# ivanalberico/End-To-End-Self-Supervised-SLAM

Hardware: AMD Instinct MI355X
Metric: online refinement steps/sec @640x480, seq_len=60 (higher is better)
Workload: dtype f32

## Files before the change

### end-to-end-self-supervised-slam_amd/csrc/conv.hip

```cpp
#include <type_traits>

#include "e2e_common.h"

typedef float f4v __attribute__((ext_vector_type(4)));
typedef float f16v __attribute__((ext_vector_type(16)));

#define CBK 16

enum { ACT_NONE = 0, ACT_RELU = 1, ACT_ELU = 2, ACT_DISP = 3 };

struct ConvArgs {
    const float* src0;
    const float* src1;
    const float* w;
    const float* scale;
    const float* shift;
    const float* res;
    float* out;
    int B, Hs, Ws;
    int Cin, C1, up;
    int Hd, Wd;
    int Ncols, ldw;
    int KH, KW, stride, pad, pad_mode;
    int off;
// ... 1733 lines not shown
        __syncthreads();
        store_chunk();
        __syncthreads();
        if (c + 1 < c_end) load_chunk(c + 1);
        constexpr int QB = 4, NQ = 32 / QB;
        float av[2][QB], bv[2][QB][3];
        auto read_q = [&](int set, int qt) {
#pragma unroll
            for (int j = 0; j < QB; ++j) {
                const int ks = QB * qt + j, q0 = (ks >> 2) * 10 + 2 * (ks & 3);
                av[set][j] = ap[2 * ks * 32];
#pragma unroll
                for (int t = 0; t < 3; ++t) bv[set][j][t] = bp[(q0 + t) * 32];
            }
        };
        auto pin_q = [&](int set) {
#pragma unroll
            for (int j = 0; j < QB; ++j) {
                asm volatile("" : "+v"(av[set][j]));
#pragma unroll
                for (int t = 0; t < 3; ++t) asm volatile("" : "+v"(bv[set][j][t]));
            }
        };
        read_q(0, 0);
#pragma unroll
        for (int qt = 0; qt < NQ; ++qt) {
            if (qt + 1 < NQ) read_q((qt + 1) & 1, qt + 1);
            __builtin_amdgcn_sched_barrier(0);
            pin_q(qt & 1);
            __builtin_amdgcn_sched_barrier(0);
#pragma unroll
            for (int j = 0; j < QB; ++j) {
#pragma unroll
                for (int t = 0; t < 3; ++t) acc[t] = __builtin_amdgcn_mfma_f32_32x32x2f32(av[qt & 1][j], bv[qt & 1][j][t], acc[t], 0, 0, 0);
                if (BIAS && want_bias) accb = __builtin_amdgcn_mfma_f32_32x32x2f32(av[qt & 1][j], one, accb, 0, 0, 0);
            }
            __builtin_amdgcn_sched_barrier(0);
        }
    }
    float* slab = a.slabs + (int64_t)blockIdx.z * a.Mpad * a.Npad;
#pragma unroll
    for (int t = 0; t < 3; ++t)
#pragma unroll
        for (int r = 0; r < 16; ++r) {
            const int m = co0 + (r & 3) + 8 * (r >> 2) + 4 * kh_;
            slab[(int64_t)m * a.Npad + (wave * 3 + t) * a.Cin + ci0 + l32] = acc[t][r];
        }
    if (BIAS && want_bias && l32 == 0) {
#pragma unroll
        for (int r = 0; r < 16; ++r) slab[(int64_t)(co0 + (r & 3) + 8 * (r >> 2) + 4 * kh_) * a.Npad + 9 * a.Cin] = accb[r];
    }
}

template <int ZL>
__device__ __forceinline__ void wgrad_reduce_group(const float* __restrict__ slabs, int S, int Mpad, int Npad, int Cout, int Cin, int KH, int KW, int has_bias,
                                                   float* __restrict__ dw, float* __restrict__ dbias, int accumulate, const float* __restrict__ scale,
                                                   int64_t base, int e, int w, f4v (*part)[64]) {
    const int Kconv = KH * KW * Cin, Ng = Kconv + (has_bias ? 1 : 0);
    const int nq = (Ng + 3) / 4;
    const int64_t totalq = (int64_t)Cout * nq;
    const int64_t slab_q = (int64_t)Mpad * Npad / 4;
    const f4v zero = {0.f, 0.f, 0.f, 0.f};
    const int64_t q = base + e;
    const bool on = q < totalq;
    const int m = on ? (int)(q / nq) : 0, n = on ? (int)(q - (int64_t)m * nq) * 4 : 0;
    const f4v* src = (const f4v*)(slabs + (int64_t)m * Npad + n);
    f4v sacc = zero;
    int z = w;
    for (; z + 3 * ZL < S; z += 4 * ZL) {
        f4v v[4];
#pragma unroll
        for (int j = 0; j < 4; ++j) v[j] = on ? src[(int64_t)(z + ZL * j) * slab_q] : zero;
#pragma unroll
        for (int j = 0; j < 4; ++j) sacc += v[j];
    }
    for (; z < S; z += ZL) sacc += on ? src[(int64_t)z * slab_q] : zero;
    part[w][e] = sacc;
    __syncthreads();
    if (w == 0 && on) {
        f4v t = part[0][e];
#pragma unroll
        for (int j = 1; j < ZL; ++j) t += part[j][e];
        if (scale) t *= scale[m];
#pragma unroll
        for (int k = 0; k < 4; ++k) {
            const int nn = n + k;
            if (nn < Kconv) {
                const int tap = nn / Cin, ci = nn - tap * Cin, kh = tap / KW, kw = tap - kh * KW;
                float* d = dw + (((int64_t)m * Cin + ci) * KH + kh) * KW + kw;
                *d = accumulate ? *d + t[k] : t[k];
            } else if (nn == Kconv && dbias) {
                dbias[m] = accumulate ? dbias[m] + t[k] : t[k];
            }
        }
    }
    __syncthreads();
}

template <int ZL>
__global__ __launch_bounds__(64 * ZL) void k_wgrad_reduce(const float* __restrict__ slabs, int S, int Mpad, int Npad, int Cout, int Cin,
                                                         int KH, int KW, int has_bias, float* __restrict__ dw, float* __restrict__ dbias,
                                                         int accumulate, const float* __restrict__ scale) {
    __shared__ f4v part[ZL][64];
    const int64_t totalq = (int64_t)Cout * ((KH * KW * Cin + (has_bias ? 1 : 0) + 3) / 4);
    for (int64_t base = (int64_t)blockIdx.x * 64; base < totalq; base += (int64_t)gridDim.x * 64)
        wgrad_reduce_group<ZL>(slabs, S, Mpad, Npad, Cout, Cin, KH, KW, has_bias, dw, dbias, accumulate, scale, base, threadIdx.x & 63, threadIdx.x >> 6, part);
}

__global__ __launch_bounds__(512) void k_wgrad_reduce_batched(const e2e_wgrad_reduce_desc* __restrict__ d, int n, long long total_items) {
    __shared__ f4v part[8][64];
    const int e = threadIdx.x & 63, w = threadIdx.x >> 6;
    for (long long item = blockIdx.x; item < total_items; item += gridDim.x) {
        int lo = 0, hi = n - 1;
        while (lo < hi) {
            const int mid = (lo + hi + 1) >> 1;
            if (d[mid].first_item <= item) lo = mid; else hi = mid - 1;
        }
        const e2e_wgrad_reduce_desc D = d[lo];
        const long long local = item - D.first_item;
        if (D.zl == 8)
            wgrad_reduce_group<8>(D.slabs, D.S, D.Mpad, D.Npad, D.Cout, D.Cin, D.KH, D.KW, D.has_bias, D.dw, D.dbias, D.accumulate, D.scale, local * 64, e, w, part);
        else
            wgrad_reduce_group<2>(D.slabs, D.S, D.Mpad, D.Npad, D.Cout, D.Cin, D.KH, D.KW, D.has_bias, D.dw, D.dbias, D.accumulate, D.scale,
                                  (local * 4 + (w >> 1)) * 64, e, w & 1, part + 2 * (w >> 1));
    }
}

__global__ __launch_bounds__(256) void k_weight_layouts(const float* __restrict__ w, int Cout, int Cin, int KH, int KW,
                                                        float* __restrict__ wf, int ldf, float* __restrict__ wb, int ldb) {
    const int64_t total = (int64_t)Cout * Cin * KH * KW;
    for (int64_t i = (int64_t)blockIdx.x * 256 + threadIdx.x; i < total; i += (int64_t)gridDim.x * 256) {
        int64_t t = i;
        const int kw = (int)(t % KW); t /= KW;
        const int kh = (int)(t % KH); t /= KH;
        const int ci = (int)(t % Cin); t /= Cin;
        const int co = (int)t;
        const float v = w[i];
        if (wf) wf[((int64_t)(kh * KW + kw) * Cin + ci) * ldf + co] = v;
        if (wb) wb[((int64_t)(kh * KW + kw) * Cout + co) * ldb + ci] = v;
    }
}

__global__ __launch_bounds__(256) void k_weight_layouts_batched(const long long* __restrict__ desc) {
    const long long* d = desc + (int64_t)blockIdx.y * 10;
    const float* __restrict__ w = (const float*)d[0];
    float* __restrict__ wf = (float*)d[1];
    float* __restrict__ wb = (float*)d[2];
    const int Cout = (int)d[3], Cin = (int)d[4], KH = (int)d[5], KW = (int)d[6], ldf = (int)d[7], ldb = (int)d[8];
    const float* __restrict__ bsc = (const float*)d[9];
    const int T = KH * KW;
    constexpr int TMAX = 9, TS = 32;
    __shared__ float tile[TMAX][TS + 1][TS + 1];
    if (T > TMAX) {
        const int64_t total = (int64_t)Cout * Cin * T;
        for (int64_t i = (int64_t)blockIdx.x * 256 + threadIdx.x; i < total; i += (int64_t)gridDim.x * 256) {
            const int tap = (int)(i % T);
            const int64_t r = i / T;
            const int ci = (int)(r % Cin), co = (int)(r / Cin);
            const float v = w[i];
            if (wf) wf[((int64_t)tap * Cin + ci) * ldf + co] = v;
            if (wb) wb[((int64_t)tap * Cout + co) * ldb + ci] = bsc ? v * bsc[co] : v;
        }
        return;
    }
    const int nct = (Cout + TS - 1) / TS, nit = (Cin + TS - 1) / TS;
    for (int t = blockIdx.x; t < nct * nit; t += gridDim.x) {
        const int co0 = (t / nit) * TS, ci0 = (t % nit) * TS;
        const int nci = min(TS, Cin - ci0), nco = min(TS, Cout - co0);
        const int row = nci * T;
        for (int e = threadIdx.x; e < nco * row; e += 256) {
            const int co_l = e / row, rem = e - co_l * row;
            const int ci_l = rem / T, tap = rem - ci_l * T;
            tile[tap][co_l][ci_l] = w[((int64_t)(co0 + co_l) * Cin + ci0) * T + rem];
        }
        __syncthreads();
        if (wf)
            for (int e = threadIdx.x; e < T * nci * nco; e += 256) {
                const int co_l = e % nco, r = e / nco;
                const int ci_l = r % nci, tap = r / nci;
                wf[((int64_t)tap * Cin + ci0 + ci_l) * ldf + co0 + co_l] = tile[tap][co_l][ci_l];
            }
        if (wb)
            for (int e = threadIdx.x; e < T * nco * nci; e += 256) {
                const int ci_l = e % nci, r = e / nci;
                const int co_l = r % nco, tap = r / nco;
                wb[((int64_t)tap * Cout + co0 + co_l) * ldb + ci0 + ci_l] = bsc ? tile[tap][co_l][ci_l] * bsc[co0 + co_l] : tile[tap][co_l][ci_l];
            }
        __syncthreads();
    }
}

__global__ __launch_bounds__(256) void k_act_bwd(const float* __restrict__ dy, const float* __restrict__ y, const float* __restrict__ scale,
                                                 float* __restrict__ dz, int64_t n, int C, int act, int accumulate) {
    for (int64_t i = (int64_t)blockIdx.x * 256 + threadIdx.x; i < n; i += (int64_t)gridDim.x * 256) {
        float g = dy[i];
        const float v = y[i];
        if (act == ACT_RELU) g = v > 0.f ? g : 0.f;
        else if (act == ACT_ELU) g = v > 0.f ? g : g * (v + 1.f);
        else if (act == ACT_DISP) { const float s = (v - 0.01f) * 0.1f; g = g * 10.f * s * (1.f - s); }
        if (scale) g *= scale[i % C];
        dz[i] = accumulate ? dz[i] + g : g;
    }
}

__global__ __launch_bounds__(256) void k_gather_adjoint(const float* __restrict__ dxp, int B, int Hs, int Ws, int Cin, int C1, int up,
                                                        int pp, float* __restrict__ d0, float* __restrict__ d1, int acc0, int acc1,
                                                        const float* __restrict__ x0, int act0, const float* __restrict__ x1, int act1) {
    const int Hp = Hs + 2 * pp, Wp = Ws + 2 * pp, C2 = Cin - C1, Hl = Hs / up, Wl = Ws / up;
    const int64_t n0 = (int64_t)B * Hl * Wl * C1, n1 = (int64_t)B * Hs * Ws * C2;
    for (int64_t i = (int64_t)blockIdx.x * 256 + threadIdx.x; i < n0 + n1; i += (int64_t)gridDim.x * 256) {
        const bool first = i < n0;
        int64_t t = first ? i : i - n0;
        const int Cx = first ? C1 : C2, Hx = first ? Hl : Hs, Wx = first ? Wl : Ws, u = first ? up : 1;
        const int c = (int)(t % Cx); t /= Cx;
        const int x = (int)(t % Wx); t /= Wx;
        const int y = (int)(t % Hx); t /= Hx;
        const int b = (int)t;
        const int cc = first ? c : C1 + c;
        float s = 0.f;
        for (int dy = 0; dy < u; ++dy)
            for (int dx = 0; dx < u; ++dx) {
                const int fy = y * u + dy, fx = x * u + dx;
                int ys[3] = {fy + pp, -1, -1}, xs[3] = {fx + pp, -1, -1};
                if (pp) {
                    if (fy == 1) ys[1] = 0;
                    if (fy == Hs - 2) ys[2] = Hp - 1;
                    if (fx == 1) xs[1] = 0;
                    if (fx == Ws - 2) xs[2] = Wp - 1;
                }
                for (int iy = 0; iy < 3; ++iy)
                    for (int ix = 0; ix < 3; ++ix)
                        if (ys[iy] >= 0 && xs[ix] >= 0) s += dxp[(((int64_t)b * Hp + ys[iy]) * Wp + xs[ix]) * Cin + cc];
            }
        float* d = first ? d0 + i : d1 + (i - n0);
        const int acc = first ? acc0 : acc1;
        if (first ? act0 : act1) s *= act_deriv(first ? x0[i] : x1[i - n0], first ? act0 : act1);
        *d = acc ? *d + s : s;
    }
}

__global__ __launch_bounds__(256) void k_gather_adjoint4(const float* __restrict__ dxp, int B, int Hs, int Ws, int Cin, int C1, int up,
// ... 281 lines not shown
            a.act == ACT_NONE) {
            a.ksplit = 4; a.cps = a.Cin / cb; a.cls_rows = Nc;
            dim3 g((unsigned)(4 * ((Nc + c.bm - 1) / c.bm)), (unsigned)((a.Ncols + c.bn - 1) / c.bn), 4u);
            launch_tile<TR>(a, cb, c, g, st);
            hipLaunchKernelGGL(k_conv_splitk_epilogue_cls, dim3(egrid(total / 4)), dim3(256), 0, st, workspace, Nc, a.B, a.Hd, a.Wd, a.Ncols, a.KH, a.KW, a.off,
                               a.res, a.out, a.xin, a.dact, a.pre);
            return;
        }
        dim3 g((unsigned)(4 * ((Nc + c.bm - 1) / c.bm)), (unsigned)((a.Ncols + c.bn - 1) / c.bn));
        launch_tile<TR>(a, cb, c, g, st);
        return;
    }
    const GemmCfg c = choose_cfg(Ntot, a.Ncols, K, cb, workspace != nullptr, force);
    if (c.S < 0 && workspace && vec == 4 && K % cb == 0 && a.Cin % cb == 0) {
        launch_streamk<TR>(a, cb, -c.S, workspace_all, st);
        return;
    }
    if (c.S > 1) {
        const int nchunks = (K + cb - 1) / cb;
        a.cps = (nchunks + c.S - 1) / c.S;
        const int Sz = (nchunks + a.cps - 1) / a.cps;
        a.ksplit = Sz;
        if (Sz > 1) {
            dim3 g((unsigned)((Ntot + c.bm - 1) / c.bm), (unsigned)((a.Ncols + c.bn - 1) / c.bn), (unsigned)Sz);
            launch_tile<TR>(a, cb, c, g, st);
            const int64_t total = Ntot * a.Ncols;
            if (a.Ncols % 4 == 0 && total < (1ll << 31))
                hipLaunchKernelGGL(k_conv_splitk_epilogue4, dim3(egrid(total / 4)), dim3(256), 0, st, workspace, Sz, (unsigned)(total / 4), a.Ncols, a.scale, a.shift,
                                   a.res, a.out, a.act, a.xin, a.dact, a.pre);
            else
                hipLaunchKernelGGL(k_conv_splitk_epilogue, dim3(egrid(total)), dim3(256), 0, st, workspace, Sz, total, a.Ncols, a.scale, a.shift, a.res, a.out, a.act, a.xin, a.dact, a.pre);
            return;
        }
        a.ksplit = 1; a.cps = 0;
    }
    dim3 g((unsigned)((Ntot + c.bm - 1) / c.bm), (unsigned)((a.Ncols + c.bn - 1) / c.bn));
    launch_tile<TR>(a, cb, c, g, st);
}

extern "C" {

int e2e_conv_weight_layouts(const float* w, int Cout, int Cin, int KH, int KW, float* w_fwd, int ld_fwd, float* w_bwd,
                            int ld_bwd, void* stream) {
    E2E_REQUIRE(w && Cout > 0 && Cin > 0 && KH > 0 && KW > 0 && (w_fwd || w_bwd), E2E_ERR_ARG, "e2e_conv_weight_layouts: bad argument");
    E2E_REQUIRE((!w_fwd || (ld_fwd >= Cout && ld_fwd % 4 == 0)) && (!w_bwd || (ld_bwd >= Cin && ld_bwd % 4 == 0)), E2E_ERR_ARG,
                "e2e_conv_weight_layouts: leading dimensions must cover the columns and be multiples of 4");
    hipLaunchKernelGGL(k_weight_layouts, dim3(egrid((int64_t)Cout * Cin * KH * KW)), dim3(256), 0, (hipStream_t)stream, w, Cout, Cin, KH,
                       KW, w_fwd, ld_fwd, w_bwd, ld_bwd);
    E2E_LAUNCH_CHECK("e2e_conv_weight_layouts");
    return E2E_OK;
}

int e2e_conv_weight_layouts_batched(const long long* desc, int nlayers, void* stream) {
    E2E_REQUIRE(desc && nlayers > 0 && nlayers <= 65535, E2E_ERR_ARG, "e2e_conv_weight_layouts_batched: bad argument");
    hipLaunchKernelGGL(k_weight_layouts_batched, dim3(256, nlayers), dim3(256), 0, (hipStream_t)stream, desc);
    E2E_LAUNCH_CHECK("e2e_conv_weight_layouts_batched");
    return E2E_OK;
}

int64_t e2e_conv2d_splitk_workspace_floats(int64_t rows, int cols, int K);
int64_t e2e_conv2d_bwd_data_workspace_floats(int B, int Hd, int Wd, int cols, int K, int stride) {
    const int64_t plain = e2e_conv2d_splitk_workspace_floats((int64_t)B * Hd * Wd, cols, K);
    if (stride != 2) return plain;
    const int64_t cls = SK_FLAG_FLOATS + (int64_t)16 * B * ((Hd + 1) / 2) * ((Wd + 1) / 2) * cols;
    return cls > plain ? cls : plain;
}

int64_t e2e_conv2d_splitk_workspace_floats(int64_t rows, int cols, int K) {
    if (K % 16 != 0) return 0;
    int smax = 1;
    bool sk = false;
    for (int cb = 16; cb <= 32; cb += 16) {
        const GemmCfg c = choose_cfg(rows, cols, K, cb, true);
        if (c.S > smax) smax = c.S;
        if (c.S < 0) sk = true;
    }
    int64_t n = smax > 1 ? (int64_t)smax * rows * cols : 0;
    if (sk && n < (int64_t)SK_MAX_G * 64 * 64) n = (int64_t)SK_MAX_G * 64 * 64;
    return n ? n + SK_FLAG_FLOATS : 0;
}

int64_t e2e_conv_tuned_workspace_floats(int64_t rows, int cols) {
    int64_t n = (int64_t)16 * rows * cols;
    if (n < (int64_t)SK_MAX_G * 64 * 64) n = (int64_t)SK_MAX_G * 64 * 64;
    return n + SK_FLAG_FLOATS;
}
int e2e_conv_workspace_flag_floats(void) { return SK_FLAG_FLOATS; }
int e2e_conv_streamk_error_index(void) { return SK_ERR_INDEX; }

int e2e_conv_gemm_choice(int64_t rows, int cols, int K, int chunk_depth, int allow_split, int* out3) {
    E2E_REQUIRE(out3 && rows > 0 && cols > 0 && K > 0 && (chunk_depth == 16 || chunk_depth == 32), E2E_ERR_ARG, "e2e_conv_gemm_choice: bad argument");
    const GemmCfg c = choose_cfg(rows, cols, K, chunk_depth, allow_split != 0);
    out3[0] = c.bm; out3[1] = c.bn; out3[2] = c.S;
    return E2E_OK;
}

static int conv_fwd_impl(const float* src0, const float* src1, int C1, int up, const float* w_fwd, int ld_fwd, const float* scale,
                         const float* shift, const float* residual, float* out, int B, int Hs, int Ws, int Cin, int Cout, int KH,
                         int KW, int stride, int pad, int pad_mode, int act, float in_sub, float in_mul, float* workspace, GemmCfg force, void* stream) {
    E2E_REQUIRE(src0 && w_fwd && out && B > 0 && Hs > 0 && Ws > 0 && Cin > 0 && Cout > 0, E2E_ERR_ARG, "e2e_conv2d_fwd: bad argument");
    E2E_REQUIRE(up == 1 || up == 2, E2E_ERR_ARG, "e2e_conv2d_fwd: upsample factor must be 1 or 2");
    E2E_REQUIRE(C1 > 0 && C1 <= Cin && (C1 == Cin || src1), E2E_ERR_ARG, "e2e_conv2d_fwd: bad channel split");
    E2E_REQUIRE(pad_mode == 0 || (pad_mode == 1 && pad == 1 && Hs >= 2 && Ws >= 2), E2E_ERR_ARG, "e2e_conv2d_fwd: reflection padding needs pad == 1");
    E2E_REQUIRE(stride == 1 || stride == 2, E2E_ERR_ARG, "e2e_conv2d_fwd: stride must be 1 or 2");
    E2E_REQUIRE(Hs % up == 0 && Ws % up == 0 && ld_fwd % 4 == 0 && ld_fwd >= Cout, E2E_ERR_ARG, "e2e_conv2d_fwd: bad sizes");
    const int vec = (Cin % 16 == 0 && (C1 == Cin || C1 % 16 == 0)) ? 4 : 1;
    E2E_REQUIRE(vec == 4 || (C1 == Cin && up == 1), E2E_ERR_ARG, "e2e_conv2d_fwd: the scalar path (Cin %% 16 != 0) takes a single full-resolution source");
    E2E_REQUIRE((int64_t)B * Hs * Ws * Cin * 4 < (1ll << 30) && (int64_t)KH * KW * Cin * ld_fwd * 4 < (1ll << 31), E2E_ERR_ARG,
// ... 226 lines not shown
    static const int target = getenv("E2E_TAP_TARGET") ? atoi(getenv("E2E_TAP_TARGET")) : TAP_TARGET;
    int S = (target + tiles - 1) / tiles;
    if (S > p.nchunks) S = p.nchunks;
    if (S < 1) S = 1;
    p.cps = (p.nchunks + S - 1) / S;
    p.S = (p.nchunks + p.cps - 1) / p.cps;
    p.Npad = (9 * Cin + (has_bias ? 1 : 0) + 3) / 4 * 4;
    return p;
}

int64_t e2e_conv2d_wgrad_workspace_floats(int B, int Ho, int Wo, int Cin, int Cout, int KH, int KW, int has_bias) {
    const WgradPlan p = wgrad_plan(B, Ho, Wo, Cin, Cout, KH, KW, has_bias, false);
    int64_t n = p.S * (int64_t)p.Mpad * p.Npad;
    if (tap_wgrad_shape_ok(Cin, Cout, KH, KW)) {
        const TapWgradPlan t = tap_wgrad_plan(B, Ho, Wo, Cin, Cout, has_bias);
        if ((int64_t)t.S * Cout * t.Npad > n) n = (int64_t)t.S * Cout * t.Npad;
    }
    if (Cout == 16) {
        const WgradPlan q = wgrad_plan(B, Ho, Wo, Cin, Cout, KH, KW, has_bias, true);
        if (q.S * (int64_t)q.Mpad * q.Npad > n) n = q.S * (int64_t)q.Mpad * q.Npad;
    }
    if (thin_wgrad_ok(Cin, Cout, KH, KW)) {
        const ThinWgradPlan t = thin_wgrad_plan(B, Ho, Wo, Cin, has_bias);
        if (t.S * Cout * t.npad > n) n = t.S * Cout * t.npad;
    }
    if (KH == 7 && KW == 7 && Cin == 3 && Cout == 64) {
        const int64_t S = (int64_t)B * ((Ho + 3) / 4) * (((Wo + 31) / 32 + 1) / 2);
        if (S * 64 * 148 > n) n = S * 64 * 148;
    }
    return n;
}

static int bwd_weight_impl(const float* dz, const float* src0, const float* src1, int C1, int up, float* dw, float* dbias, float* workspace, int B,
                           int Hs, int Ws, int Cin, int Cout, int Ho, int Wo, int KH, int KW, int stride, int pad, int pad_mode, int accumulate,
                           float in_sub, float in_mul, const float* out_scale, void* stream, int wg_target = 0, e2e_wgrad_reduce_desc* defer = nullptr) {
    const bool tuned = wg_target != 0;
    if (!tuned) wg_target = WGRAD_TARGET;
    E2E_REQUIRE(dz && src0 && dw && workspace && B > 0 && Cin > 0 && Cout > 0, E2E_ERR_ARG, "e2e_conv2d_bwd_weight: bad argument");
    const int vec = (Cin % 4 == 0 && C1 % 4 == 0) ? 4 : 1;
    E2E_REQUIRE(vec == 4 || (C1 == Cin && up == 1 && pad_mode == 0), E2E_ERR_ARG, "e2e_conv2d_bwd_weight: scalar path takes one full-resolution zero-padded source");
    WgradArgs a{};
    a.dz = dz; a.src0 = src0; a.src1 = src1; a.slabs = workspace;
    a.B = B; a.Hs = Hs; a.Ws = Ws; a.Cin = Cin; a.C1 = C1; a.up = up; a.Ho = Ho; a.Wo = Wo; a.Cout = Cout;
    a.KH = KH; a.KW = KW; a.stride = stride; a.pad = pad; a.pad_mode = pad_mode; a.has_bias = dbias ? 1 : 0;
    a.Ngemm = KH * KW * Cin + a.has_bias;
    const int64_t P = (int64_t)B * Ho * Wo;
    const bool lean = vec == 4 && Cout % 4 == 0 && Wo >= 8 && (int64_t)B * Hs * Ws * Cin * 4 < (1ll << 31) && P * Cout * 4 < (1ll << 31) && P < (1ll << 24);
    hipStream_t st = (hipStream_t)stream;
    auto reduce = [&](int S, int Mpad, int Npad, int zl) {
        if (defer) {
            *defer = e2e_wgrad_reduce_desc{workspace, dw, dbias, out_scale, S, Mpad, Npad, Cout, Cin, KH, KW, a.has_bias, accumulate, zl, 0};
            return;
        }
        const int64_t tq = (int64_t)Cout * ((a.Ngemm + 3) / 4);
        if (zl == 8)
            hipLaunchKernelGGL((k_wgrad_reduce<8>), dim3(egrid(tq * 4)), dim3(512), 0, st, workspace, S, Mpad, Npad, Cout, Cin, KH, KW, a.has_bias, dw, dbias,
                               accumulate, out_scale);
        else
            hipLaunchKernelGGL((k_wgrad_reduce<2>), dim3(egrid(tq * 4)), dim3(128), 0, st, workspace, S, Mpad, Npad, Cout, Cin, KH, KW, a.has_bias, dw, dbias,
                               accumulate, out_scale);
    };
    if (KH == 7 && KW == 7 && stride == 2 && pad == 3 && pad_mode == 0 && Cin == 3 && Cout == 64 && C1 == Cin && up == 1 && !dbias &&
        Ho == (Hs + 6 - 7) / 2 + 1 && Wo == (Ws + 6 - 7) / 2 + 1) {
        const int nxg = ((Wo + 31) / 32 + 1) / 2, ny = (Ho + 3) / 4;
        StemWgradArgs ta{dz, src0, workspace, B, Hs, Ws, Ho, Wo, 2, nxg, in_sub, in_mul};
        hipLaunchKernelGGL(k_wgrad7x7_stem, dim3(nxg, ny, B), dim3(256), 0, st, ta);
        reduce(B * ny * nxg, 64, 148, 8);
        E2E_LAUNCH_CHECK("e2e_conv2d_bwd_weight");
        return E2E_OK;
    }
    if (!tuned && lean && thin_wgrad_ok(Cin, Cout, KH, KW) && stride == 1 && pad == 1 && pad_mode == 1 && C1 % 16 == 0 && Ho == Hs && Wo == Ws &&
        (C1 == Cin || src1) && Hs % up == 0 && Ws % up == 0) {
        const ThinWgradPlan t = thin_wgrad_plan(B, Ho, Wo, Cin, a.has_bias);
        ThinWgradArgs ta{dz, src0, src1, workspace, B, Ho, Wo, Cin, C1, up, t.npad, a.has_bias, t.tiles_x, t.nxg};
        const dim3 tg((unsigned)t.nxg, (unsigned)t.ny, (unsigned)(B * (Cin / 16)));
        if (Cout == 32) hipLaunchKernelGGL((k_wgrad3x3_thin<2>), tg, dim3(256), 0, st, ta);
        else hipLaunchKernelGGL((k_wgrad3x3_thin<1>), tg, dim3(256), 0, st, ta);
        reduce((int)t.S, Cout, t.npad, 8);
        E2E_LAUNCH_CHECK("e2e_conv2d_bwd_weight");
        return E2E_OK;
    }
    if (!tuned && vec == 4 && tap_wgrad_shape_ok(Cin, Cout, KH, KW) && stride == 1 && pad == 1 && Ho == Hs && Wo == Ws && (up == 1 || up == 2) &&
        Hs % up == 0 && Ws % up == 0 && (C1 == Cin || (src1 && C1 % 32 == 0)) && getenv("E2E_WGRAD_TAPS") != nullptr && getenv("E2E_WGRAD_TAPS")[0] == '1') {
        const TapWgradPlan t = tap_wgrad_plan(B, Ho, Wo, Cin, Cout, a.has_bias);
        TapWgradArgs ta{dz, src0, src1, workspace, B, Ho, Wo, Cin, C1, up, Cout, pad_mode == 1 ? 1 : 0, a.has_bias, Cout, t.Npad, t.ptx, t.pty, t.nchunks, t.cps};
        const dim3 tg((unsigned)(Cin / 32), (unsigned)(Cout / 32), (unsigned)t.S);
        if (a.has_bias) hipLaunchKernelGGL(k_wgrad3x3_taps<true>, tg, dim3(TAP_NT), 0, st, ta);
        else hipLaunchKernelGGL(k_wgrad3x3_taps<false>, tg, dim3(TAP_NT), 0, st, ta);
        reduce(t.S, Cout, t.Npad, t.S >= 8 ? 8 : 2);
        E2E_LAUNCH_CHECK("e2e_conv2d_bwd_weight");
        return E2E_OK;
    }
    const bool use16 = lean && Cout == 16;
    const WgradPlan wp = wgrad_plan(B, Ho, Wo, Cin, Cout, KH, KW, a.has_bias, use16, wg_target);
    const int tm = wp.tm, tn = wp.tn;
    a.Mpad = wp.Mpad; a.Npad = wp.Npad;
    a.in_sub = in_sub; a.in_mul = in_mul; a.vec = vec;
    const int64_t S = wp.S;
    const int cbp = lean ? 32 : CBK;
    a.pix_per_slice = ((P + S - 1) / S + cbp - 1) / cbp * cbp;
    const int Sz = (int)((P + a.pix_per_slice - 1) / a.pix_per_slice);
    dim3 g((unsigned)(a.Npad / tn), (unsigned)(a.Mpad / tm), (unsigned)Sz);
    if (use16) {
        hipLaunchKernelGGL((k_wgrad_gemm16<10, 32>), g, dim3(256), 0, st, a);
    } else if (lean) {
        if (tm == 32) {
            if (src1) hipLaunchKernelGGL((k_wgrad_gemm4<1, 4, 32, true>), g, dim3(256), 0, st, a);
            else hipLaunchKernelGGL((k_wgrad_gemm4<1, 4, 32, false>), g, dim3(256), 0, st, a);
        } else {
            if (src1) hipLaunchKernelGGL((k_wgrad_gemm4<2, 2, 32, true>), g, dim3(256), 0, st, a);
            else hipLaunchKernelGGL((k_wgrad_gemm4<2, 2, 32, false>), g, dim3(256), 0, st, a);
        }
    } else if (tm == 32) {
        if (vec == 4) hipLaunchKernelGGL((k_wgrad_gemm<1, 4, 4>), g, dim3(256), 0, st, a);
        else hipLaunchKernelGGL((k_wgrad_gemm<1, 4, 1>), g, dim3(256), 0, st, a);
    } else {
        if (vec == 4) hipLaunchKernelGGL((k_wgrad_gemm<2, 2, 4>), g, dim3(256), 0, st, a);
        else hipLaunchKernelGGL((k_wgrad_gemm<2, 2, 1>), g, dim3(256), 0, st, a);
    }
    reduce(Sz, a.Mpad, a.Npad, Sz >= 8 ? 8 : 2);
    E2E_LAUNCH_CHECK("e2e_conv2d_bwd_weight");
    return E2E_OK;
}

int e2e_conv2d_bwd_weight(const float* dz, const float* src0, const float* src1, int C1, int up, float* dw, float* dbias,
                          float* workspace, int B, int Hs, int Ws, int Cin, int Cout, int Ho, int Wo, int KH, int KW, int stride,
                          int pad, int pad_mode, int accumulate, float in_sub, float in_mul, void* stream) {
    return bwd_weight_impl(dz, src0, src1, C1, up, dw, dbias, workspace, B, Hs, Ws, Cin, Cout, Ho, Wo, KH, KW, stride, pad, pad_mode, accumulate,
                           in_sub, in_mul, nullptr, stream);
}

int e2e_conv2d_bwd_weight_scaled(const float* da, const float* out_scale, const float* src0, const float* src1, int C1, int up, float* dw,
                                 float* dbias, float* workspace, int B, int Hs, int Ws, int Cin, int Cout, int Ho, int Wo, int KH, int KW,
                                 int stride, int pad, int pad_mode, int accumulate, float in_sub, float in_mul, void* stream) {
    return bwd_weight_impl(da, src0, src1, C1, up, dw, dbias, workspace, B, Hs, Ws, Cin, Cout, Ho, Wo, KH, KW, stride, pad, pad_mode, accumulate,
                           in_sub, in_mul, out_scale, stream);
}

int e2e_conv2d_bwd_weight_scaled_deferred(const float* da, const float* out_scale, const float* src0, const float* src1, int C1, int up, float* dw,
                                          float* dbias, float* workspace, int B, int Hs, int Ws, int Cin, int Cout, int Ho, int Wo, int KH, int KW,
                                          int stride, int pad, int pad_mode, int accumulate, float in_sub, float in_mul,
                                          e2e_wgrad_reduce_desc* desc_out, void* stream) {
    E2E_REQUIRE(desc_out, E2E_ERR_ARG, "e2e_conv2d_bwd_weight_scaled_deferred: desc_out is NULL");
    return bwd_weight_impl(da, src0, src1, C1, up, dw, dbias, workspace, B, Hs, Ws, Cin, Cout, Ho, Wo, KH, KW, stride, pad, pad_mode, accumulate,
                           in_sub, in_mul, out_scale, stream, 0, desc_out);
}

long long e2e_wgrad_reduce_batch_prepare(e2e_wgrad_reduce_desc* descs_host, int n) {
    if (!descs_host || n <= 0) return -1;
    long long total = 0;
    for (int i = 0; i < n; ++i) {
        e2e_wgrad_reduce_desc& d = descs_host[i];
        if (!d.slabs || !d.dw || d.S <= 0 || d.Mpad <= 0 || d.Npad <= 0 || d.Npad % 4 || d.Cout <= 0 || d.Cin <= 0 || d.KH <= 0 || d.KW <= 0 || (d.zl != 8 && d.zl != 2))
            return -1;
        const long long quads = (long long)d.Cout * ((d.KH * d.KW * d.Cin + (d.has_bias ? 1 : 0) + 3) / 4);
        d.first_item = total;
        total += (quads + (d.zl == 8 ? 63 : 255)) / (d.zl == 8 ? 64 : 256);
    }
    return total;
}

int e2e_wgrad_reduce_batched(const e2e_wgrad_reduce_desc* descs_dev, int n, long long total_items, void* stream) {
    E2E_REQUIRE(descs_dev && n > 0 && total_items > 0, E2E_ERR_ARG, "e2e_wgrad_reduce_batched: bad argument");
    hipLaunchKernelGGL(k_wgrad_reduce_batched, dim3((unsigned)(total_items < 4096 ? total_items : 4096)), dim3(512), 0, (hipStream_t)stream, descs_dev, n, total_items);
    E2E_LAUNCH_CHECK("e2e_wgrad_reduce_batched");
    return E2E_OK;
}

int e2e_conv2d_bwd_weight_scaled_tuned(const float* da, const float* out_scale, const float* src0, const float* src1, int C1, int up, float* dw,
                                       float* dbias, float* workspace, int B, int Hs, int Ws, int Cin, int Cout, int Ho, int Wo, int KH, int KW,
                                       int stride, int pad, int pad_mode, int accumulate, float in_sub, float in_mul, int target_workgroups, void* stream) {
    E2E_REQUIRE(target_workgroups >= 64 && target_workgroups <= 8192, E2E_ERR_ARG, "e2e_conv2d_bwd_weight_scaled_tuned: 64 .. 8192 workgroups");
    return bwd_weight_impl(da, src0, src1, C1, up, dw, dbias, workspace, B, Hs, Ws, Cin, Cout, Ho, Wo, KH, KW, stride, pad, pad_mode, accumulate,
                           in_sub, in_mul, out_scale, stream, target_workgroups);
}

int64_t e2e_conv2d_wgrad_tuned_workspace_floats(int B, int Ho, int Wo, int Cin, int Cout, int KH, int KW, int has_bias, int target_workgroups) {
    int64_t n = 0;
    for (int u = 0; u < 2; ++u) {
        if (u == 1 && Cout != 16) break;
        const WgradPlan p = wgrad_plan(B, Ho, Wo, Cin, Cout, KH, KW, has_bias, u == 1, target_workgroups);
        if (p.S * (int64_t)p.Mpad * p.Npad > n) n = p.S * (int64_t)p.Mpad * p.Npad;
    }
    return n;
}

#ifdef E2E_CONV_STAMPS
int e2e_debug_read_stamps(unsigned long long* host, int n) {
    if (n < -(1 << 20)) return (int)hipMemcpyFromSymbol(host, HIP_SYMBOL(g_phases), (size_t)(-n - (1 << 20)) * 8);
    if (n < 0) return (int)hipMemcpyFromSymbol(host, HIP_SYMBOL(g_stamps2), (size_t)(-n) * 8);
    return (int)hipMemcpyFromSymbol(host, HIP_SYMBOL(g_stamps), (size_t)n * 8);
}
#endif

}
```

Measured before the change: 207.7.

## Restructure wgrad slab reduction into panel/deep paths and retile batched weight layout kernel

Replaces the per-quad split-K weight-gradient reduction with two strategies. A panel path reduces whole output-channel rows in shared memory and writes dw contiguously with vector stores. A deep path stages many slabs through LDS with register prefetch. Both the single and batched reducers now share this plan. The batched weight-layout transpose kernel is also rewritten to use a flat tile list across layers, tap-specialized tiles and vectorized loads/stores. This adds a large shared-memory footprint (about 64KB per block), which could lower occupancy.

```diff
diff --git a/end-to-end-self-supervised-slam_amd/csrc/conv.hip b/end-to-end-self-supervised-slam_amd/csrc/conv.hip
--- a/end-to-end-self-supervised-slam_amd/csrc/conv.hip
+++ b/end-to-end-self-supervised-slam_amd/csrc/conv.hip
@@ -1809,45 +1809,84 @@
     }
 }
 
+#define WRED_DEEP_S 32
+#define WRED_PANEL 8192
+#define WRED_ITEM_BYTES (128 << 10)
+struct WredPlan { int deep, r, nq; long long items; };
+__host__ __device__ inline WredPlan wred_plan(int S, int Cout, int Cin, int KH, int KW, int has_bias) {
+    WredPlan p;
+    const int Kconv = KH * KW * Cin;
+    p.nq = (Kconv + (has_bias ? 1 : 0) + 3) / 4;
+    p.deep = S >= WRED_DEEP_S || Kconv > WRED_PANEL;
+    if (p.deep) {
+        p.r = 0;
+        p.items = ((long long)Cout * p.nq + 7) / 8;
+        return p;
+    }
+    long long r = WRED_PANEL / Kconv;
+    const long long rw = WRED_ITEM_BYTES / ((long long)p.nq * 16 * S);
+    if (rw < r) r = rw;
+    if (r > Cout) r = Cout;
+    if (r < 1) r = 1;
+    p.r = (int)r;
+    p.items = (Cout + p.r - 1) / p.r;
+    return p;
+}
+
+struct WredSmem {
+    f4v buf[2048];
+    float panel[WRED_PANEL];
+};
+
 template <int ZL>
-__device__ __forceinline__ void wgrad_reduce_group(const float* __restrict__ slabs, int S, int Mpad, int Npad, int Cout, int Cin, int KH, int KW, int has_bias,
-                                                   float* __restrict__ dw, float* __restrict__ dbias, int accumulate, const float* __restrict__ scale,
-                                                   int64_t base, int e, int w, f4v (*part)[64]) {
-    const int Kconv = KH * KW * Cin, Ng = Kconv + (has_bias ? 1 : 0);
-    const int nq = (Ng + 3) / 4;
-    const int64_t totalq = (int64_t)Cout * nq;
-    const int64_t slab_q = (int64_t)Mpad * Npad / 4;
+__device__ __forceinline__ void wgrad_reduce_deep(const e2e_wgrad_reduce_desc& D, const WredPlan& P, long long item, WredSmem& sm) {
+    const int tid = threadIdx.x, j = tid & 7, s = tid >> 3;
+    const int Kconv = D.KH * D.KW * D.Cin, nq = P.nq;
+    const int64_t slab = (int64_t)D.Mpad * D.Npad;
     const f4v zero = {0.f, 0.f, 0.f, 0.f};
-    const int64_t q = base + e;
-    const bool on = q < totalq;
-    const int m = on ? (int)(q / nq) : 0, n = on ? (int)(q - (int64_t)m * nq) * 4 : 0;
-    const f4v* src = (const f4v*)(slabs + (int64_t)m * Npad + n);
-    f4v sacc = zero;
-    int z = w;
-    for (; z + 3 * ZL < S; z += 4 * ZL) {
-        f4v v[4];
-#pragma unroll
-        for (int j = 0; j < 4; ++j) v[j] = on ? src[(int64_t)(z + ZL * j) * slab_q] : zero;
-#pragma unroll
-        for (int j = 0; j < 4; ++j) sacc += v[j];
-    }
-    for (; z < S; z += ZL) sacc += on ? src[(int64_t)z * slab_q] : zero;
-    part[w][e] = sacc;
+    const long long q = item * 8 + j;
+    const bool on = q < (long long)D.Cout * nq;
+    const int m = on ? (int)(q / nq) : 0, n = on ? (int)(q - (long long)m * nq) * 4 : 0;
+    const float* src = D.slabs + (int64_t)m * D.Npad + n;
+    f4v v[4];
+#pragma unroll
+    for (int k = 0; k < 4; ++k) v[k] = (on && s + 64 * k < D.S) ? *(const f4v*)(src + (int64_t)(s + 64 * k) * slab) : zero;
+    const bool chain = tid < 8 * ZL;
+    const int cq = tid & 7, zw = tid >> 3;
+    f4v p = zero;
+    for (int base = 0; base < D.S; base += 256) {
+#pragma unroll
+        for (int k = 0; k < 4; ++k) sm.buf[tid + 512 * k] = v[k];
+        __syncthreads();
+        if (base + 256 < D.S) {
+#pragma unroll
+            for (int k = 0; k < 4; ++k) {
+                const int z = base + 256 + s + 64 * k;
+                v[k] = (on && z < D.S) ? *(const f4v*)(src + (int64_t)z * slab) : zero;
+            }
+        }
+        if (chain) {
+            const int zn = min(256, D.S - base);
+            for (int zz = zw; zz < zn; zz += ZL) p += sm.buf[zz * 8 + cq];
+        }
+        __syncthreads();
+    }
+    if (chain) sm.buf[tid] = p;
     __syncthreads();
-    if (w == 0 && on) {
-        f4v t = part[0][e];
-#pragma unroll
-        for (int j = 1; j < ZL; ++j) t += part[j][e];
-        if (scale) t *= scale[m];
+    if (tid < 8 && on) {
+        f4v t = sm.buf[tid];
+#pragma unroll
+        for (int w = 1; w < ZL; ++w) t += sm.buf[w * 8 + tid];
+        if (D.scale) t *= D.scale[m];
 #pragma unroll
         for (int k = 0; k < 4; ++k) {
             const int nn = n + k;
             if (nn < Kconv) {
-                const int tap = nn / Cin, ci = nn - tap * Cin, kh = tap / KW, kw = tap - kh * KW;
-                float* d = dw + (((int64_t)m * Cin + ci) * KH + kh) * KW + kw;
-                *d = accumulate ? *d + t[k] : t[k];
-            } else if (nn == Kconv && dbias) {
-                dbias[m] = accumulate ? dbias[m] + t[k] : t[k];
+                const int tap = nn / D.Cin, ci = nn - tap * D.Cin, kh = tap / D.KW, kw = tap - kh * D.KW;
+                float* d = D.dw + (((int64_t)m * D.Cin + ci) * D.KH + kh) * D.KW + kw;
+                *d = D.accumulate ? *d + t[k] : t[k];
+            } else if (nn == Kconv && D.dbias) {
+                D.dbias[m] = D.accumulate ? D.dbias[m] + t[k] : t[k];
             }
         }
     }
@@ -1855,18 +1894,95 @@
 }
 
 template <int ZL>
-__global__ __launch_bounds__(64 * ZL) void k_wgrad_reduce(const float* __restrict__ slabs, int S, int Mpad, int Npad, int Cout, int Cin,
-                                                         int KH, int KW, int has_bias, float* __restrict__ dw, float* __restrict__ dbias,
-                                                         int accumulate, const float* __restrict__ scale) {
-    __shared__ f4v part[ZL][64];
-    const int64_t totalq = (int64_t)Cout * ((KH * KW * Cin + (has_bias ? 1 : 0) + 3) / 4);
-    for (int64_t base = (int64_t)blockIdx.x * 64; base < totalq; base += (int64_t)gridDim.x * 64)
-        wgrad_reduce_group<ZL>(slabs, S, Mpad, Npad, Cout, Cin, KH, KW, has_bias, dw, dbias, accumulate, scale, base, threadIdx.x & 63, threadIdx.x >> 6, part);
+__device__ __forceinline__ void wgrad_reduce_panel(const e2e_wgrad_reduce_desc& D, const WredPlan& P, long long item, WredSmem& sm) {
+    constexpr int G = 8 / ZL, U = 4, CQ = 64 * G * U;
+    const int tid = threadIdx.x, e = tid & 63, w = tid >> 6, zw = w % ZL, g = w / ZL;
+    const int T = D.KH * D.KW, Kconv = T * D.Cin, nq = P.nq;
+    const int m0 = (int)item * P.r, rows = min(P.r, D.Cout - m0), Q = rows * nq;
+    const int64_t slab = (int64_t)D.Mpad * D.Npad;
+    const f4v zero = {0.f, 0.f, 0.f, 0.f};
+    const float* base = D.slabs + (int64_t)m0 * D.Npad;
+    for (int c0 = 0; c0 < Q; c0 += CQ) {
+        const float* src[U];
+        bool on[U];
+        f4v acc[U];
+#pragma unroll
+        for (int u = 0; u < U; ++u) {
+            const int q = c0 + g * 64 + e + 64 * G * u;
+            on[u] = q < Q;
+            const int mr = on[u] ? q / nq : 0, n = on[u] ? (q - mr * nq) * 4 : 0;
+            src[u] = base + (int64_t)mr * D.Npad + n;
+            acc[u] = zero;
+        }
+        int z = zw;
+        for (; z + ZL < D.S; z += 2 * ZL) {
+            f4v a[U], b[U];
+#pragma unroll
+            for (int u = 0; u < U; ++u) {
+                a[u] = on[u] ? *(const f4v*)(src[u] + (int64_t)z * slab) : zero;
+                b[u] = on[u] ? *(const f4v*)(src[u] + (int64_t)(z + ZL) * slab) : zero;
+            }
+#pragma unroll
+            for (int u = 0; u < U; ++u) acc[u] += a[u];
+#pragma unroll
+            for (int u = 0; u < U; ++u) acc[u] += b[u];
+        }
+        if (z < D.S) {
+#pragma unroll
+            for (int u = 0; u < U; ++u) acc[u] += on[u] ? *(const f4v*)(src[u] + (int64_t)z * slab) : zero;
+        }
+#pragma unroll
+        for (int u = 0; u < U; ++u) sm.buf[zw * CQ + g * 64 + e + 64 * G * u] = acc[u];
+        __syncthreads();
+        for (int lq = tid; lq < CQ; lq += 512) {
+            const int q = c0 + lq;
+            if (q >= Q) break;
+            const int mr = q / nq, n = (q - mr * nq) * 4;
+            f4v t = sm.buf[lq];
+#pragma unroll
+            for (int k = 1; k < ZL; ++k) t += sm.buf[k * CQ + lq];
+            if (D.scale) t *= D.scale[m0 + mr];
+            int tap = n / D.Cin, ci = n - tap * D.Cin;
+#pragma unroll
+            for (int k = 0; k < 4; ++k) {
+                if (n + k < Kconv) sm.panel[mr * Kconv + ci * T + tap] = t[k];
+                else if (n + k == Kconv && D.dbias) D.dbias[m0 + mr] = D.accumulate ? D.dbias[m0 + mr] + t[k] : t[k];
+                if (++ci == D.Cin) { ci = 0; ++tap; }
+            }
+        }
+        __syncthreads();
+    }
+    float* dst = D.dw + (int64_t)m0 * Kconv;
+    const int len = rows * Kconv;
+    int i0 = 0;
+    if ((reinterpret_cast<uintptr_t>(dst) & 15) == 0) {
+        const f4v* pv = (const f4v*)sm.panel;
+        f4v* dv = (f4v*)dst;
+        for (int i = tid; i < len / 4; i += 512) dv[i] = D.accumulate ? dv[i] + pv[i] : pv[i];
+        i0 = len / 4 * 4;
+    }
+    for (int i = i0 + tid; i < len; i += 512) dst[i] = D.accumulate ? dst[i] + sm.panel[i] : sm.panel[i];
+    __syncthreads();
+}
+
+__device__ __forceinline__ void wgrad_reduce_item(const e2e_wgrad_reduce_desc& D, long long item, WredSmem& sm) {
+    const WredPlan P = wred_plan(D.S, D.Cout, D.Cin, D.KH, D.KW, D.has_bias);
+    if (P.deep) {
+        if (D.zl == 8) wgrad_reduce_deep<8>(D, P, item, sm);
+        else wgrad_reduce_deep<2>(D, P, item, sm);
+    } else {
+        if (D.zl == 8) wgrad_reduce_panel<8>(D, P, item, sm);
+        else wgrad_reduce_panel<2>(D, P, item, sm);
+    }
+}
+
+__global__ __launch_bounds__(512) void k_wgrad_reduce(const e2e_wgrad_reduce_desc D, long long items) {
+    __shared__ WredSmem sm;
+    for (long long item = blockIdx.x; item < items; item += gridDim.x) wgrad_reduce_item(D, item, sm);
 }
 
 __global__ __launch_bounds__(512) void k_wgrad_reduce_batched(const e2e_wgrad_reduce_desc* __restrict__ d, int n, long long total_items) {
-    __shared__ f4v part[8][64];
-    const int e = threadIdx.x & 63, w = threadIdx.x >> 6;
+    __shared__ WredSmem sm;
     for (long long item = blockIdx.x; item < total_items; item += gridDim.x) {
         int lo = 0, hi = n - 1;
         while (lo < hi) {
@@ -1874,12 +1990,7 @@
             if (d[mid].first_item <= item) lo = mid; else hi = mid - 1;
         }
         const e2e_wgrad_reduce_desc D = d[lo];
-        const long long local = item - D.first_item;
-        if (D.zl == 8)
-            wgrad_reduce_group<8>(D.slabs, D.S, D.Mpad, D.Npad, D.Cout, D.Cin, D.KH, D.KW, D.has_bias, D.dw, D.dbias, D.accumulate, D.scale, local * 64, e, w, part);
-        else
-            wgrad_reduce_group<2>(D.slabs, D.S, D.Mpad, D.Npad, D.Cout, D.Cin, D.KH, D.KW, D.has_bias, D.dw, D.dbias, D.accumulate, D.scale,
-                                  (local * 4 + (w >> 1)) * 64, e, w & 1, part + 2 * (w >> 1));
+        wgrad_reduce_item(D, item - D.first_item, sm);
     }
 }
 
@@ -1898,52 +2009,121 @@
     }
 }
 
-__global__ __launch_bounds__(256) void k_weight_layouts_batched(const long long* __restrict__ desc) {
-    const long long* d = desc + (int64_t)blockIdx.y * 10;
-    const float* __restrict__ w = (const float*)d[0];
-    float* __restrict__ wf = (float*)d[1];
-    float* __restrict__ wb = (float*)d[2];
-    const int Cout = (int)d[3], Cin = (int)d[4], KH = (int)d[5], KW = (int)d[6], ldf = (int)d[7], ldb = (int)d[8];
-    const float* __restrict__ bsc = (const float*)d[9];
-    const int T = KH * KW;
-    constexpr int TMAX = 9, TS = 32;
-    __shared__ float tile[TMAX][TS + 1][TS + 1];
-    if (T > TMAX) {
-        const int64_t total = (int64_t)Cout * Cin * T;
-        for (int64_t i = (int64_t)blockIdx.x * 256 + threadIdx.x; i < total; i += (int64_t)gridDim.x * 256) {
-            const int tap = (int)(i % T);
-            const int64_t r = i / T;
-            const int ci = (int)(r % Cin), co = (int)(r / Cin);
-            const float v = w[i];
-            if (wf) wf[((int64_t)tap * Cin + ci) * ldf + co] = v;
-            if (wb) wb[((int64_t)tap * Cout + co) * ldb + ci] = bsc ? v * bsc[co] : v;
-        }
-        return;
-    }
-    const int nct = (Cout + TS - 1) / TS, nit = (Cin + TS - 1) / TS;
-    for (int t = blockIdx.x; t < nct * nit; t += gridDim.x) {
-        const int co0 = (t / nit) * TS, ci0 = (t % nit) * TS;
-        const int nci = min(TS, Cin - ci0), nco = min(TS, Cout - co0);
-        const int row = nci * T;
-        for (int e = threadIdx.x; e < nco * row; e += 256) {
-            const int co_l = e / row, rem = e - co_l * row;
-            const int ci_l = rem / T, tap = rem - ci_l * T;
-            tile[tap][co_l][ci_l] = w[((int64_t)(co0 + co_l) * Cin + ci0) * T + rem];
-        }
-        __syncthreads();
-        if (wf)
-            for (int e = threadIdx.x; e < T * nci * nco; e += 256) {
-                const int co_l = e % nco, r = e / nco;
-                const int ci_l = r % nci, tap = r / nci;
-                wf[((int64_t)tap * Cin + ci0 + ci_l) * ldf + co0 + co_l] = tile[tap][co_l][ci_l];
-            }
-        if (wb)
-            for (int e = threadIdx.x; e < T * nco * nci; e += 256) {
-                const int ci_l = e % nci, r = e / nci;
-                const int co_l = r % nco, tap = r / nco;
-                wb[((int64_t)tap * Cout + co0 + co_l) * ldb + ci0 + ci_l] = bsc ? tile[tap][co_l][ci_l] * bsc[co0 + co_l] : tile[tap][co_l][ci_l];
-            }
-        __syncthreads();
+#define WL_MAX_LAYERS 1024
+#define WL_GRID 1024
+constexpr int wl_cit(int T) { return T == 9 ? 32 : T == 1 ? 32 : 4; }
+struct WlTile { const float* w; float* wf; float* wb; const float* bsc; int Cout, Cin, ldf, ldb, co0, ci0, nco, nci; };
+
+template <int T>
+__device__ __forceinline__ void weight_layout_tile(const WlTile& t, float* img) {
+    constexpr int CIT = wl_cit(T), RS = CIT * T + 1, RL = CIT * T;
+    const int tid = threadIdx.x;
+    const int len = t.nci * T;
+    const float* src = t.w + ((int64_t)t.co0 * t.Cin + t.ci0) * T;
+    const int64_t rstride = (int64_t)t.Cin * T;
+    if ((len & 3) == 0 && (rstride & 3) == 0 && (reinterpret_cast<uintptr_t>(src) & 15) == 0) {
+        constexpr int NV = RL / 4;
+        for (int i = tid; i < 32 * NV; i += 256) {
+            const int co_l = i / NV, qq = i - co_l * NV;
+            if (co_l < t.nco && qq * 4 < len) {
+                const f4v v = *(const f4v*)(src + co_l * rstride + qq * 4);
+#pragma unroll
+                for (int k = 0; k < 4; ++k) img[co_l * RS + qq * 4 + k] = v[k];
+            }
+        }
+    } else {
+        for (int i = tid; i < 32 * RL; i += 256) {
+            const int co_l = i / RL, r = i - co_l * RL;
+            if (co_l < t.nco && r < len) img[co_l * RS + r] = src[co_l * rstride + r];
+        }
+    }
+    __syncthreads();
+    if (t.wf) {
+        float* dst = t.wf + ((int64_t)t.ci0) * t.ldf + t.co0;
+        if ((t.nco & 3) == 0 && (t.ldf & 3) == 0 && (reinterpret_cast<uintptr_t>(dst) & 15) == 0) {
+            for (int i = tid; i < T * CIT * 8; i += 256) {
+                const int cq = i & 7, r = i >> 3, ci_l = r % CIT, tap = r / CIT;
+                if (ci_l < t.nci && cq * 4 < t.nco) {
+                    const int o = cq * 4 * RS + ci_l * T + tap;
+                    const f4v v = {img[o], img[o + RS], img[o + 2 * RS], img[o + 3 * RS]};
+                    *(f4v*)(dst + ((int64_t)tap * t.Cin + ci_l) * t.ldf + cq * 4) = v;
+                }
+            }
+        } else {
+            for (int i = tid; i < T * CIT * 32; i += 256) {
+                const int co_l = i & 31, r = i >> 5, ci_l = r % CIT, tap = r / CIT;
+                if (ci_l < t.nci && co_l < t.nco) dst[((int64_t)tap * t.Cin + ci_l) * t.ldf + co_l] = img[co_l * RS + ci_l * T + tap];
+            }
+        }
+    }
+    if (t.wb) {
+        float* dst = t.wb + ((int64_t)t.co0) * t.ldb + t.ci0;
+        if (CIT % 4 == 0 && (t.nci & 3) == 0 && (t.ldb & 3) == 0 && (reinterpret_cast<uintptr_t>(dst) & 15) == 0) {
+            constexpr int NQ = CIT / 4 > 0 ? CIT / 4 : 1;
+            for (int i = tid; i < T * 32 * NQ; i += 256) {
+                const int iq = i % NQ, r = i / NQ, co_l = r & 31, tap = r >> 5;
+                if (co_l < t.nco && iq * 4 < t.nci) {
+                    const int o = co_l * RS + iq * 4 * T + tap;
+                    f4v v = {img[o], img[o + T], img[o + 2 * T], img[o + 3 * T]};
+                    if (t.bsc) v *= t.bsc[t.co0 + co_l];
+                    *(f4v*)(dst + ((int64_t)tap * t.Cout + co_l) * t.ldb + iq * 4) = v;
+                }
+            }
+        } else {
+            for (int i = tid; i < T * 32 * CIT; i += 256) {
+                const int ci_l = i % CIT, r = i / CIT, co_l = r & 31, tap = r >> 5;
+                if (co_l < t.nco && ci_l < t.nci) {
+                    const float v = img[co_l * RS + ci_l * T + tap];
+                    dst[((int64_t)tap * t.Cout + co_l) * t.ldb + ci_l] = t.bsc ? v * t.bsc[t.co0 + co_l] : v;
+                }
+            }
+        }
+    }
+    __syncthreads();
+}
+
+__global__ __launch_bounds__(256) void k_weight_layouts_batched(const long long* __restrict__ desc, int nlayers) {
+    __shared__ int first[WL_MAX_LAYERS + 1];
+    __shared__ float img[32 * (wl_cit(9) * 9 + 1)];
+    for (int l = threadIdx.x; l < nlayers; l += 256) {
+        const long long* d = desc + (int64_t)l * 10;
+        const int Cout = (int)d[3], Cin = (int)d[4], T = (int)(d[5] * d[6]);
+        const int cit = T == 9 || T == 1 ? 32 : T == 49 ? 4 : 1;
+        first[l + 1] = ((Cout + 31) / 32) * ((Cin + cit - 1) / cit);
+    }
+    __syncthreads();
+    if (threadIdx.x == 0) {
+        first[0] = 0;
+        for (int l = 0; l < nlayers; ++l) first[l + 1] += first[l];
+    }
+    __syncthreads();
+    const int total = first[nlayers];
+    for (int tile = blockIdx.x; tile < total; tile += gridDim.x) {
+        int lo = 0, hi = nlayers - 1;
+        while (lo < hi) {
+            const int mid = (lo + hi + 1) >> 1;
+            if (first[mid] <= tile) lo = mid; else hi = mid - 1;
+        }
+        const long long* d = desc + (int64_t)lo * 10;
+        WlTile t;
+        t.w = (const float*)d[0]; t.wf = (float*)d[1]; t.wb = (float*)d[2]; t.bsc = (const float*)d[9];
+        t.Cout = (int)d[3]; t.Cin = (int)d[4]; t.ldf = (int)d[7]; t.ldb = (int)d[8];
+        const int T = (int)(d[5] * d[6]);
+        const int cit = T == 9 || T == 1 ? 32 : T == 49 ? 4 : 1;
+        const int nit = (t.Cin + cit - 1) / cit, local = tile - first[lo];
+        t.co0 = (local / nit) * 32; t.ci0 = (local - (local / nit) * nit) * cit;
+        t.nco = min(32, t.Cout - t.co0); t.nci = min(cit, t.Cin - t.ci0);
+        if (T == 9) weight_layout_tile<9>(t, img);
+        else if (T == 1) weight_layout_tile<1>(t, img);
+        else if (T == 49) weight_layout_tile<49>(t, img);
+        else {
+            for (int i = threadIdx.x; i < t.nco * T; i += 256) {
+                const int co_l = i / T, tap = i - co_l * T, co = t.co0 + co_l;
+                const float v = t.w[((int64_t)co * t.Cin + t.ci0) * T + tap];
+                if (t.wf) t.wf[((int64_t)tap * t.Cin + t.ci0) * t.ldf + co] = v;
+                if (t.wb) t.wb[((int64_t)tap * t.Cout + co) * t.ldb + t.ci0] = t.bsc ? v * t.bsc[co] : v;
+            }
+        }
     }
 }
 
@@ -2331,8 +2511,8 @@
 }
 
 int e2e_conv_weight_layouts_batched(const long long* desc, int nlayers, void* stream) {
-    E2E_REQUIRE(desc && nlayers > 0 && nlayers <= 65535, E2E_ERR_ARG, "e2e_conv_weight_layouts_batched: bad argument");
-    hipLaunchKernelGGL(k_weight_layouts_batched, dim3(256, nlayers), dim3(256), 0, (hipStream_t)stream, desc);
+    E2E_REQUIRE(desc && nlayers > 0 && nlayers <= WL_MAX_LAYERS, E2E_ERR_ARG, "e2e_conv_weight_layouts_batched: bad argument");
+    hipLaunchKernelGGL(k_weight_layouts_batched, dim3(WL_GRID), dim3(256), 0, (hipStream_t)stream, desc, nlayers);
     E2E_LAUNCH_CHECK("e2e_conv_weight_layouts_batched");
     return E2E_OK;
 }
@@ -2665,13 +2845,9 @@
             *defer = e2e_wgrad_reduce_desc{workspace, dw, dbias, out_scale, S, Mpad, Npad, Cout, Cin, KH, KW, a.has_bias, accumulate, zl, 0};
             return;
         }
-        const int64_t tq = (int64_t)Cout * ((a.Ngemm + 3) / 4);
-        if (zl == 8)
-            hipLaunchKernelGGL((k_wgrad_reduce<8>), dim3(egrid(tq * 4)), dim3(512), 0, st, workspace, S, Mpad, Npad, Cout, Cin, KH, KW, a.has_bias, dw, dbias,
-                               accumulate, out_scale);
-        else
-            hipLaunchKernelGGL((k_wgrad_reduce<2>), dim3(egrid(tq * 4)), dim3(128), 0, st, workspace, S, Mpad, Npad, Cout, Cin, KH, KW, a.has_bias, dw, dbias,
-                               accumulate, out_scale);
+        const e2e_wgrad_reduce_desc D{workspace, dw, dbias, out_scale, S, Mpad, Npad, Cout, Cin, KH, KW, a.has_bias, accumulate, zl, 0};
+        const long long items = wred_plan(S, Cout, Cin, KH, KW, a.has_bias).items;
+        hipLaunchKernelGGL(k_wgrad_reduce, dim3((unsigned)(items < 4096 ? items : 4096)), dim3(512), 0, st, D, items);
     };
     if (KH == 7 && KW == 7 && stride == 2 && pad == 3 && pad_mode == 0 && Cin == 3 && Cout == 64 && C1 == Cin && up == 1 && !dbias &&
         Ho == (Hs + 6 - 7) / 2 + 1 && Wo == (Ws + 6 - 7) / 2 + 1) {
@@ -2766,9 +2942,8 @@
         e2e_wgrad_reduce_desc& d = descs_host[i];
         if (!d.slabs || !d.dw || d.S <= 0 || d.Mpad <= 0 || d.Npad <= 0 || d.Npad % 4 || d.Cout <= 0 || d.Cin <= 0 || d.KH <= 0 || d.KW <= 0 || (d.zl != 8 && d.zl != 2))
             return -1;
-        const long long quads = (long long)d.Cout * ((d.KH * d.KW * d.Cin + (d.has_bias ? 1 : 0) + 3) / 4);
         d.first_item = total;
-        total += (quads + (d.zl == 8 ? 63 : 255)) / (d.zl == 8 ? 64 : 256);
+        total += wred_plan(d.S, d.Cout, d.Cin, d.KH, d.KW, d.has_bias).items;
     }
     return total;
 }
```

Result: no change. 209.7, median of 6 (+1.0%).
